# fwrnke/pseudo-3D-interpolation

Hardware: AMD Instinct MI355X
Metric: POCS iterations/s on the 1024x1024x512 cube (higher is better)
Workload: dtype complex64 (f32 arithmetic)

## Files before the change

### include/p3d.h

```cpp
#ifndef P3D_H
#define P3D_H

#include <stddef.h>
#include <stdint.h>

#ifdef __cplusplus
extern "C" {
#endif

#define P3D_ABI_VERSION 1

#define P3D_OK 0
#define P3D_ERR_INVALID (-1)
#define P3D_ERR_UNSUPPORTED (-2)
#define P3D_ERR_HIP (-3)

#define P3D_C64 0
#define P3D_F32 1
#define P3D_C128 2
#define P3D_F64 3

#define P3D_OP_HARD 0
#define P3D_OP_SOFT 1
#define P3D_OP_GARROTE 2
#define P3D_OP_PERCENTILE 16

#define P3D_VER_REGULAR 0
#define P3D_VER_FAST 1
#define P3D_VER_ADAPTIVE 2

#define P3D_FLAG_PROFILE 1
#define P3D_FLAG_PRIMED 2
#define P3D_FLAG_MASK_PER_SLICE 4

typedef struct p3d_plan p3d_plan;

typedef struct p3d_pocs_params {
    int32_t niter;
    int32_t thresh_op;
    int32_t version;
    int32_t flags;
    double eps;
    double alpha;
} p3d_pocs_params;

#define P3D_STATS_PER_SLICE 6

int p3d_abi_version(void);
const char* p3d_last_error(void);
int p3d_runtime_info(int* compiled_hip_version, int* runtime_hip_version);
int p3d_device_count(int* n);

int p3d_shape_supported(int nil, int nxl);

int p3d_plan_create(p3d_plan** out, int device, int nil, int nxl, int max_slices);
int p3d_plan_destroy(p3d_plan* plan);

int p3d_malloc(p3d_plan* plan, void** dptr, size_t bytes);
int p3d_free(p3d_plan* plan, void* dptr);
int p3d_memcpy_h2d(p3d_plan* plan, void* dst_dev, const void* src_host, size_t bytes);
int p3d_memcpy_d2h(p3d_plan* plan, void* dst_host, const void* src_dev, size_t bytes);
int p3d_dev_malloc(int device, void** dptr, size_t bytes);
int p3d_dev_free(void* dptr);
int p3d_dev_memcpy(int device, void* dst, const void* src, size_t bytes, int kind);
int p3d_dev_memset(int device, void* dptr, int value, size_t bytes);
int p3d_dev_synchronize(int device);
int p3d_dev_mem_info(int device, size_t* free_bytes, size_t* total_bytes);
int p3d_host_alloc(void** hptr, size_t bytes);
int p3d_host_free(void* hptr);
int p3d_host_register(void* hptr, size_t bytes);
int p3d_host_unregister(void* hptr);

int p3d_fft2_c64_dev(p3d_plan* plan, const void* in_dev, void* out_dev, int nslices, int inverse);
int p3d_fft2_c64(p3d_plan* plan, const void* in_host, void* out_host, int nslices, int inverse);

int p3d_fft2_shrink_c64(p3d_plan* plan, const void* in_host, const double* tau, int thresh_op, void* out_host,
                        int nslices);

int p3d_pocs_stats_dev(p3d_plan* plan, const void* x_dev, int dtype, int nslices, double* stats_host);
int p3d_pocs_prime_dev(p3d_plan* plan, const void* x_dev, int dtype, const float* mask_dev, int nslices, double* stats_host);
int p3d_pocs_stats(p3d_plan* plan, const void* x_host, int dtype, int nslices, double* stats_host);

int p3d_pocs_sorted_spectrum(p3d_plan* plan, const void* x, int nslices, float* peaks_host);
int p3d_pocs_data_driven_pick(p3d_plan* plan, int nslices, int niter, const float* bounds_host, float* tau_host, int64_t* count_host);

int p3d_pocs_run_dev(p3d_plan* plan, const void* x_dev, int dtype, const float* mask_dev, const double* tau,
                     const uint8_t* active, const p3d_pocs_params* params, void* out_dev, int nslices,
                     int32_t* niter_done, double* sums, double* elapsed_ms);
int p3d_pocs_run(p3d_plan* plan, const void* x_host, int dtype, const float* mask_host, const double* tau,
                 const uint8_t* active, const p3d_pocs_params* params, void* out_host, int nslices,
                 int32_t* niter_done, double* sums, double* elapsed_ms);

int p3d_multi_stats(int ndev, const int* devices, int nil, int nxl, const void* x_host, int dtype, int nslices, double* stats_host);
int p3d_multi_run(int ndev, const int* devices, int nil, int nxl, const void* x_host, int dtype, const float* mask_host,
                  const double* tau, const uint8_t* active, const p3d_pocs_params* params, void* out_host, int nslices,
                  int32_t* niter_done, double* sums);

#define P3D_DCT_BACKWARD 0
#define P3D_DCT_ORTHO 1
int p3d_dct2_c64_dev(p3d_plan* plan, const void* in_dev, void* out_dev, int nslices, int inverse, int norm);
int p3d_dct2_c64(p3d_plan* plan, const void* in_host, void* out_host, int nslices, int inverse, int norm);
int p3d_dct_shrink_c64(p3d_plan* plan, const void* in_host, const double* tau, int thresh_op, void* out_host, int nslices, int norm);
int p3d_pocs_dct_stats_dev(p3d_plan* plan, const void* x_dev, int dtype, int nslices, double* stats_host, int norm);
int p3d_pocs_dct_stats(p3d_plan* plan, const void* x_host, int dtype, int nslices, double* stats_host, int norm);
int p3d_pocs_dct_run_dev(p3d_plan* plan, const void* x_dev, int dtype, const float* mask_dev, const double* tau, const uint8_t* active,
                         const p3d_pocs_params* params, void* out_dev, int nslices, int32_t* niter_done, double* sums,
                         double* elapsed_ms, int norm);
int p3d_pocs_dct_run(p3d_plan* plan, const void* x_host, int dtype, const float* mask_host, const double* tau, const uint8_t* active,
                     const p3d_pocs_params* params, void* out_host, int nslices, int32_t* niter_done, double* sums,
                     double* elapsed_ms, int norm);

typedef struct p3d_patch_plan p3d_patch_plan;
int p3d_patch_plan_create(p3d_patch_plan** out, p3d_plan* plan, int nil, int nxl, const int32_t* starts_il, int n_il, const int32_t* starts_xl,
                          int n_xl, const float* taper_il, const float* taper_xl, int max_slices);
int p3d_patch_plan_destroy(p3d_patch_plan* pplan);
int p3d_patch_plan_info(p3d_patch_plan* pplan, int* npatch, int* max_jobs, int* resident_shape);
int p3d_patch_gather_dev(p3d_patch_plan* pplan, const void* cube_dev, int dtype, int nslices, void* patches_dev);
int p3d_patch_mask_dev(p3d_patch_plan* pplan, const float* mask_dev, int mask_slices, int nslices, float* windows_dev, int* nonbinary);
int p3d_patch_route(p3d_patch_plan* pplan, const p3d_pocs_params* params, int* single_kernel);
int p3d_patch_run_dev(p3d_patch_plan* pplan, const void* patches_dev, int dtype, const double* tau, const uint8_t* active,
                      const p3d_pocs_params* params, void* out_dev, int nslices, int32_t* niter_done, double* sums, double* elapsed_ms);
int p3d_patch_dct_route(p3d_patch_plan* pplan, const p3d_pocs_params* params, int norm, int* single_kernel);
int p3d_patch_dct_run_dev(p3d_patch_plan* pplan, const void* patches_dev, int dtype, const double* tau, const uint8_t* active,
                          const p3d_pocs_params* params, int norm, void* out_dev, int nslices, int32_t* niter_done, double* sums, double* elapsed_ms);
int p3d_patch_blend_dev(p3d_patch_plan* pplan, const void* patches_dev, int dtype, const uint8_t* active, void* out_dev, int nslices);

typedef struct p3d_plan64 p3d_plan64;
int p3d_plan64_create(p3d_plan64** out, int device, int nil, int nxl, int max_slices);
int p3d_plan64_destroy(p3d_plan64* plan);
int p3d_pocs64_stats(p3d_plan64* plan, const void* x, int dtype, int nslices, double* stats_host);
int p3d_fft2_c128(p3d_plan64* plan, const void* in_host, void* out_host, int nslices, int inverse);
int p3d_pocs64_run(p3d_plan64* plan, const void* x, int dtype, const double* mask, const double* tau, const uint8_t* active,
                   const p3d_pocs_params* params, void* out, int nslices, int32_t* niter_done, double* sums, double* elapsed_ms);
int p3d_pocs64_percentile(p3d_plan64* plan, const void* spectrum_host_c128, int nslices, const double* perc_host, double* thr_host);
// ... 194 lines not shown
```

### pseudo-3d-interpolation_amd/_ffi.py

```python
import ctypes as C
import importlib.util
import os
import sys

import numpy as np

_HERE = os.path.dirname(os.path.abspath(__file__))
LIB_PATH = os.environ.get("P3D_LIB_PATH") or os.path.join(_HERE, "libp3d_hip.so")

P3D_OK = 0
P3D_ERR_INVALID, P3D_ERR_UNSUPPORTED, P3D_ERR_HIP = -1, -2, -3
P3D_C64, P3D_F32 = 0, 1
P3D_C128, P3D_F64 = 2, 3
P3D_OP = {"hard": 0, "soft": 1, "garrote": 2, "garotte": 2}
P3D_OP_PERCENTILE = 16
P3D_OP.update({f"{k}-percentile": v | P3D_OP_PERCENTILE for k, v in list(P3D_OP.items())})
P3D_VER = {"regular": 0, "fast": 1, "adaptive": 2}
P3D_FLAG_PROFILE = 1
P3D_FLAG_PRIMED = 2
P3D_FLAG_MASK_PER_SLICE = 4
STATS_PER_SLICE = 6
P3D_DCT_NORM = {None: 0, "backward": 0, "ortho": 1}


class P3DError(RuntimeError):
    def __init__(self, code, msg):
        super().__init__(f"libp3d_hip error {code}: {msg}")
        self.code = code


class UnsupportedError(P3DError, NotImplementedError):
    pass


class PocsParams(C.Structure):
    _fields_ = [("niter", C.c_int32), ("thresh_op", C.c_int32), ("version", C.c_int32), ("flags", C.c_int32),
                ("eps", C.c_double), ("alpha", C.c_double)]


_lib = None

PROTOTYPES = {
    "p3d_abi_version": (C.c_int, []),
    "p3d_last_error": (C.c_char_p, []),
    "p3d_device_count": (C.c_int, [C.POINTER(C.c_int)]),
    "p3d_shape_supported": (C.c_int, [C.c_int, C.c_int]),
    "p3d_plan_create": (C.c_int, [C.POINTER(C.c_void_p), C.c_int, C.c_int, C.c_int, C.c_int]),
    "p3d_plan_destroy": (C.c_int, [C.c_void_p]),
    "p3d_malloc": (C.c_int, [C.c_void_p, C.POINTER(C.c_void_p), C.c_size_t]),
    "p3d_free": (C.c_int, [C.c_void_p, C.c_void_p]),
    "p3d_host_alloc": (C.c_int, [C.POINTER(C.c_void_p), C.c_size_t]),
    "p3d_host_free": (C.c_int, [C.c_void_p]),
    "p3d_memcpy_h2d": (C.c_int, [C.c_void_p, C.c_void_p, C.c_void_p, C.c_size_t]),
    "p3d_memcpy_d2h": (C.c_int, [C.c_void_p, C.c_void_p, C.c_void_p, C.c_size_t]),
    "p3d_fft2_c64_dev": (C.c_int, [C.c_void_p, C.c_void_p, C.c_void_p, C.c_int, C.c_int]),
    "p3d_fft2_c64": (C.c_int, [C.c_void_p, C.c_void_p, C.c_void_p, C.c_int, C.c_int]),
    "p3d_fft2_shrink_c64": (C.c_int, [C.c_void_p, C.c_void_p, C.c_void_p, C.c_int, C.c_void_p, C.c_int]),
    "p3d_pocs_stats_dev": (C.c_int, [C.c_void_p, C.c_void_p, C.c_int, C.c_int, C.c_void_p]),
    "p3d_runtime_info": (C.c_int, [C.POINTER(C.c_int), C.POINTER(C.c_int)]),
    "p3d_plan64_create": (C.c_int, [C.POINTER(C.c_void_p), C.c_int, C.c_int, C.c_int, C.c_int]),
    "p3d_plan64_destroy": (C.c_int, [C.c_void_p]),
    "p3d_pocs64_stats": (C.c_int, [C.c_void_p, C.c_void_p, C.c_int, C.c_int, C.c_void_p]),
    "p3d_fft2_c128": (C.c_int, [C.c_void_p, C.c_void_p, C.c_void_p, C.c_int, C.c_int]),
    "p3d_pocs64_run": (C.c_int, [C.c_void_p, C.c_void_p, C.c_int, C.c_void_p, C.c_void_p, C.c_void_p, C.POINTER(PocsParams), C.c_void_p, C.c_int,
                                 C.c_void_p, C.c_void_p, C.POINTER(C.c_double)]),
    "p3d_pocs64_percentile": (C.c_int, [C.c_void_p, C.c_void_p, C.c_int, C.c_void_p, C.c_void_p]),
    "p3d_pocs64_sorted_spectrum": (C.c_int, [C.c_void_p, C.c_void_p, C.c_int, C.c_int, C.c_void_p]),
    "p3d_pocs64_data_driven_pick": (C.c_int, [C.c_void_p, C.c_int, C.c_int, C.c_void_p, C.c_void_p, C.c_void_p]),
    "p3d_dct2_c128": (C.c_int, [C.c_void_p, C.c_void_p, C.c_void_p, C.c_int, C.c_int, C.c_int]),
    "p3d_pocs64_dct_stats": (C.c_int, [C.c_void_p, C.c_void_p, C.c_int, C.c_int, C.c_void_p, C.c_int]),
    "p3d_pocs64_dct_run": (C.c_int, [C.c_void_p, C.c_void_p, C.c_int, C.c_void_p, C.c_void_p, C.c_void_p, C.POINTER(PocsParams), C.c_void_p, C.c_int,
                                     C.c_void_p, C.c_void_p, C.POINTER(C.c_double), C.c_int]),
    "p3d_dev_malloc": (C.c_int, [C.c_int, C.POINTER(C.c_void_p), C.c_size_t]),
    "p3d_dev_free": (C.c_int, [C.c_void_p]),
    "p3d_dev_memcpy": (C.c_int, [C.c_int, C.c_void_p, C.c_void_p, C.c_size_t, C.c_int]),
    "p3d_dev_memset": (C.c_int, [C.c_int, C.c_void_p, C.c_int, C.c_size_t]),
    "p3d_dev_synchronize": (C.c_int, [C.c_int]),
    "p3d_dev_mem_info": (C.c_int, [C.c_int, C.POINTER(C.c_size_t), C.POINTER(C.c_size_t)]),
    "p3d_host_register": (C.c_int, [C.c_void_p, C.c_size_t]),
    "p3d_host_unregister": (C.c_int, [C.c_void_p]),
    "p3d_pocs_prime_dev": (C.c_int, [C.c_void_p, C.c_void_p, C.c_int, C.c_void_p, C.c_int, C.c_void_p]),
    "p3d_pocs_stats": (C.c_int, [C.c_void_p, C.c_void_p, C.c_int, C.c_int, C.c_void_p]),
    "p3d_pocs_sorted_spectrum": (C.c_int, [C.c_void_p, C.c_void_p, C.c_int, C.c_void_p]),
    "p3d_pocs_data_driven_pick": (C.c_int, [C.c_void_p, C.c_int, C.c_int, C.c_void_p, C.c_void_p, C.c_void_p]),
    "p3d_pocs_run_dev": (C.c_int, [C.c_void_p, C.c_void_p, C.c_int, C.c_void_p, C.c_void_p, C.c_void_p,
                                   C.POINTER(PocsParams), C.c_void_p, C.c_int, C.c_void_p, C.c_void_p,
                                   C.POINTER(C.c_double)]),
    "p3d_dct2_c64_dev": (C.c_int, [C.c_void_p, C.c_void_p, C.c_void_p, C.c_int, C.c_int, C.c_int]),
    "p3d_dct2_c64": (C.c_int, [C.c_void_p, C.c_void_p, C.c_void_p, C.c_int, C.c_int, C.c_int]),
    "p3d_dct_shrink_c64": (C.c_int, [C.c_void_p, C.c_void_p, C.c_void_p, C.c_int, C.c_void_p, C.c_int, C.c_int]),
    "p3d_pocs_dct_stats_dev": (C.c_int, [C.c_void_p, C.c_void_p, C.c_int, C.c_int, C.c_void_p, C.c_int]),
    "p3d_pocs_dct_stats": (C.c_int, [C.c_void_p, C.c_void_p, C.c_int, C.c_int, C.c_void_p, C.c_int]),
    "p3d_pocs_dct_run_dev": (C.c_int, [C.c_void_p, C.c_void_p, C.c_int, C.c_void_p, C.c_void_p, C.c_void_p,
                                   C.POINTER(PocsParams), C.c_void_p, C.c_int, C.c_void_p, C.c_void_p,
                                   C.POINTER(C.c_double), C.c_int]),
    "p3d_pocs_dct_run": (C.c_int, [C.c_void_p, C.c_void_p, C.c_int, C.c_void_p, C.c_void_p, C.c_void_p,
                                   C.POINTER(PocsParams), C.c_void_p, C.c_int, C.c_void_p, C.c_void_p,
                                   C.POINTER(C.c_double), C.c_int]),
    "p3d_pocs_run": (C.c_int, [C.c_void_p, C.c_void_p, C.c_int, C.c_void_p, C.c_void_p, C.c_void_p,
                               C.POINTER(PocsParams), C.c_void_p, C.c_int, C.c_void_p, C.c_void_p,
                               C.POINTER(C.c_double)]),
    "p3d_patch_plan_create": (C.c_int, [C.POINTER(C.c_void_p), C.c_void_p, C.c_int, C.c_int, C.c_void_p, C.c_int, C.c_void_p, C.c_int, C.c_void_p, C.c_void_p,
                                        C.c_int]),
    "p3d_patch_plan_destroy": (C.c_int, [C.c_void_p]),
    "p3d_patch_plan_info": (C.c_int, [C.c_void_p, C.POINTER(C.c_int), C.POINTER(C.c_int), C.POINTER(C.c_int)]),
    "p3d_patch_gather_dev": (C.c_int, [C.c_void_p, C.c_void_p, C.c_int, C.c_int, C.c_void_p]),
    "p3d_patch_mask_dev": (C.c_int, [C.c_void_p, C.c_void_p, C.c_int, C.c_int, C.c_void_p, C.POINTER(C.c_int)]),
    "p3d_patch_route": (C.c_int, [C.c_void_p, C.POINTER(PocsParams), C.POINTER(C.c_int)]),
    "p3d_patch_run_dev": (C.c_int, [C.c_void_p, C.c_void_p, C.c_int, C.c_void_p, C.c_void_p, C.POINTER(PocsParams), C.c_void_p, C.c_int, C.c_void_p,
                                    C.c_void_p, C.POINTER(C.c_double)]),
    "p3d_patch_dct_route": (C.c_int, [C.c_void_p, C.POINTER(PocsParams), C.c_int, C.POINTER(C.c_int)]),
    "p3d_patch_dct_run_dev": (C.c_int, [C.c_void_p, C.c_void_p, C.c_int, C.c_void_p, C.c_void_p, C.POINTER(PocsParams), C.c_int, C.c_void_p, C.c_int, C.c_void_p,
                                        C.c_void_p, C.POINTER(C.c_double)]),
    "p3d_patch_blend_dev": (C.c_int, [C.c_void_p, C.c_void_p, C.c_int, C.c_void_p, C.c_void_p, C.c_int]),
    "p3d_multi_stats": (C.c_int, [C.c_int, C.c_void_p, C.c_int, C.c_int, C.c_void_p, C.c_int, C.c_int, C.c_void_p]),
    "p3d_multi_run": (C.c_int, [C.c_int, C.c_void_p, C.c_int, C.c_int, C.c_void_p, C.c_int, C.c_void_p, C.c_void_p, C.c_void_p,
                                C.POINTER(PocsParams), C.c_void_p, C.c_int, C.c_void_p, C.c_void_p]),
    "p3d_time2freq": (C.c_int, [C.c_int, C.c_void_p, C.c_int, C.c_size_t, C.c_double, C.c_double, C.c_int, C.c_int, C.c_void_p,
                                C.c_void_p]),
    "p3d_freq2time": (C.c_int, [C.c_int, C.c_void_p, C.c_int, C.c_void_p, C.c_size_t, C.c_double, C.c_double, C.c_int, C.c_int,
                                C.c_void_p]),
    "p3d_time2freq_dev": (C.c_int, [C.c_int, C.c_void_p, C.c_int, C.c_size_t, C.c_double, C.c_double, C.c_int, C.c_int, C.c_void_p,
                                    C.c_void_p]),
    "p3d_freq2time_dev": (C.c_int, [C.c_int, C.c_void_p, C.c_int, C.c_void_p, C.c_size_t, C.c_double, C.c_double, C.c_int, C.c_int,
                                    C.c_void_p]),
    "p3d_last_sparsity": (C.c_int, [C.c_void_p, C.POINTER(C.c_double)]),
    "p3d_smooth_gaussian": (C.c_int, [C.c_int, C.c_void_p, C.c_size_t, C.c_int, C.c_int, C.c_double, C.c_double, C.c_void_p]),
    "p3d_smooth_median": (C.c_int, [C.c_int, C.c_void_p, C.c_size_t, C.c_int, C.c_int, C.c_int, C.c_void_p]),
# ... 89 lines not shown
    "p3d_shearlet_transform_c64": (C.c_int, [C.c_void_p, C.c_void_p, C.c_void_p, C.c_int]),
    "p3d_shearlet_inverse_c64": (C.c_int, [C.c_void_p, C.c_void_p, C.c_void_p, C.c_int]),
    "p3d_shearlet_stats": (C.c_int, [C.c_void_p, C.c_void_p, C.c_int, C.c_int, C.c_void_p]),
    "p3d_shearlet_run": (C.c_int, [C.c_void_p, C.c_void_p, C.c_int, C.c_void_p, C.c_void_p, C.c_void_p, C.POINTER(PocsParams),
                                   C.c_void_p, C.c_int, C.c_void_p, C.c_void_p, C.POINTER(C.c_double)]),
}


def _preload_torch_hip():
    if not os.environ.get("P3D_TORCH_HIP_PRELOAD") or "torch" in sys.modules:
        return
    try:
        spec = importlib.util.find_spec("torch")
        path = os.path.join(os.path.dirname(spec.origin), "lib", "libamdhip64.so") if spec and spec.origin else None
        if path and os.path.isfile(path):
            C.CDLL(path, mode=C.RTLD_GLOBAL)
    except (ImportError, OSError, ValueError):
        pass


def lib():
    global _lib
    if _lib is None:
        if not os.path.isfile(LIB_PATH):
            raise ImportError(
                f"{LIB_PATH} not found: build it with `make -C {os.path.join(_HERE, 'csrc')}` "
                "(or python -c 'import __graft_entry__ as g; g.build()'). There is no CPU fallback.")
        _preload_torch_hip()
        handle = C.CDLL(LIB_PATH)
        for name, (res, args) in PROTOTYPES.items():
            fn = getattr(handle, name)
            fn.restype = res
            fn.argtypes = args
        _lib = handle
        _check_runtime(handle)
    return _lib


_runtime = None


def _check_runtime(handle):
    global _runtime
    comp, run = C.c_int(0), C.c_int(0)
    path = None
    try:
        if handle.p3d_runtime_info(C.byref(comp), C.byref(run)) != P3D_OK:
            return
        with open("/proc/self/maps") as fh:
            for line in fh:
                if "libamdhip64" in line:
                    path = line.split()[-1]
                    break
    except OSError:
        pass

    def split(v):
        return v // 10000000, (v // 100000) % 100, v % 100000
    _runtime = {"compiled_hip_version": "%d.%d.%d" % split(comp.value), "runtime_hip_version": "%d.%d.%d" % split(run.value), "runtime_library": path}
    if split(comp.value)[:2] != split(run.value)[:2]:
        import warnings
        warnings.warn(f"libp3d_hip.so was compiled against HIP {_runtime['compiled_hip_version']} but the process runs HIP "
                      f"{_runtime['runtime_hip_version']} ({path}): another copy of the runtime was mapped first (PyTorch imported before this package, or "
                      f"P3D_TORCH_HIP_PRELOAD=1); processes that do not need torch.cuda should load this package first", RuntimeWarning, stacklevel=3)


def runtime_info():
    lib()
    return dict(_runtime or {})


def check(code):
    if code != P3D_OK:
        msg = lib().p3d_last_error().decode("utf-8", "replace")
        raise (UnsupportedError if code == P3D_ERR_UNSUPPORTED else P3DError)(code, msg)


def device_count():
    n = C.c_int(0)
    check(lib().p3d_device_count(C.byref(n)))
    return n.value


def shape_supported(nil, nxl):
    return bool(lib().p3d_shape_supported(int(nil), int(nxl)))


def _ptr(a):
    return a.ctypes.data_as(C.c_void_p)


class DeviceBuffer:

    def __init__(self, plan, nbytes):
        self.plan, self.nbytes = plan, int(nbytes)
        p = C.c_void_p()
        check(lib().p3d_malloc(plan.handle, C.byref(p), self.nbytes))
        self.ptr = p.value

    def upload(self, arr):
        arr = np.ascontiguousarray(arr)
        assert arr.nbytes <= self.nbytes
        check(lib().p3d_memcpy_h2d(self.plan.handle, self.ptr, _ptr(arr), arr.nbytes))
        return self

    def download(self, shape, dtype):
        out = np.empty(shape, dtype)
        assert out.nbytes <= self.nbytes
        check(lib().p3d_memcpy_d2h(self.plan.handle, _ptr(out), self.ptr, out.nbytes))
        return out

    def download_into(self, arr):
        if not arr.flags.c_contiguous or arr.nbytes > self.nbytes:
            raise ValueError("destination must be C-contiguous and no larger than the buffer")
        check(lib().p3d_memcpy_d2h(self.plan.handle, _ptr(arr), self.ptr, arr.nbytes))
        return arr

    def free(self):
        if self.ptr:
            check(lib().p3d_free(self.plan.handle, self.ptr))
            self.ptr = None


def _tau_table(tau, shape):
    tau = np.broadcast_to(np.asarray(tau), shape)
    t = np.empty(tau.shape + (2,), np.float64)
    t[..., 0] = tau.real
    t[..., 1] = tau.imag if np.iscomplexobj(tau) else 0.0
    return t


def _filter_bank(wavelet):
    bank = wavelet if isinstance(wavelet, (tuple, list)) else wavelet_filters(wavelet)
    bank = [np.ascontiguousarray(b, dtype=np.float64) for b in bank]
    if len(bank) != 4 or len({b.size for b in bank}) != 1:
        raise ValueError("a filter bank is (dec_lo, dec_hi, rec_lo, rec_hi) of equal length")
    return bank


def _real_psi(psi):
    psi = np.asarray(psi)
    if psi.ndim != 3:
        raise ValueError(f"Psi must be (nil, nxl, nshearlets), got shape {psi.shape}")
    if np.iscomplexobj(psi):
        raise NotImplementedError("complex shearlet spectra (realCoefficients=False) are not implemented")
    return psi


class _PlanBase:
    _DESTROY = _RUN = None
    _MASK_DT = np.float32

    def close(self):
        if getattr(self, "handle", None):
            getattr(lib(), self._DESTROY)(self.handle)
            self.handle = None

    def __del__(self):
        if lib is not None:
            self.close()

    def __enter__(self):
        return self

    def __exit__(self, *exc):
        self.close()
# ... 1410 lines not shown
```

### pseudo-3d-interpolation_amd/csrc/p3d_api.hip

```cpp
#include <hip/hip_runtime.h>

#include <climits>
#include <cmath>
#include <algorithm>
#include <cstdlib>
#include <cstring>
#include <string>
#include <thread>
#include <vector>

#include "p3d.h"
#include "p3d_dct.hpp"
#include "p3d_dct_tables.hpp"
#include "p3d_generic.hpp"
#include "p3d_host.hpp"
#include "p3d_internal.hpp"
#include "p3d_flex.hpp"
#include "p3d_mix_entry.hpp"
#include "p3d_resident.hpp"
#include "p3d_resident_dct.hpp"
#include "p3d_select.hpp"
#include "p3d_kernels.hpp"

namespace p3d {
// ... 280 lines not shown
    unsigned long long* nzl = nullptr;
    unsigned* cbase = nullptr;
    unsigned long long* mbits = nullptr;
    unsigned* mbase = nullptr;
    const p3d::mix::Entry* mix_row = nullptr;
    bool mix_binary = false;
    bool use32 = false;
    unsigned long long* bits32 = nullptr;
    c32* tw32 = nullptr;
    int* flag = nullptr;
    unsigned* rowbase = nullptr;
    char* xc = nullptr;
    size_t xc_cap = 0;
    double* sums = nullptr;
    size_t sums_cap = 0;
    double* rowsum = nullptr;
    c32* tau = nullptr;
    size_t tau_cap = 0;
    int* done = nullptr;
    float* partials = nullptr;
    int tiles = 0;
    int cus = 0;
    int pipe_wgs = 0;
    int host_sw = 0;
    int flex_over = 0;
    bool no_colpipe = false;
    void* st_x = nullptr;
    void* st_out = nullptr;
    float* st_mask = nullptr;
    size_t st_mask_cap = 0;
    size_t st_cap = 0;
    struct Primed { bool valid = false; const void* x = nullptr; const float* mask = nullptr; int dtype = 0, nslices = 0, nonbinary = 0, violation = 0; unsigned nobs = 0;
                    bool real = false;
    } primed;
    double* sum0 = nullptr;
    int sorted_slices = 0;
    c32* dct_w = nullptr;
    c32* dct_tab = nullptr;
    hipEvent_t ev0 = nullptr, ev1 = nullptr;
    std::vector<hipEvent_t> prof_events;
    double prof_col_ms = 0, prof_row_ms = 0;
    int prof_col_n = 0, prof_row_n = 0;

    size_t slice_elems() const { return (size_t)nil * nxl; }
};

static int upload_table(p3d_plan* p, const LineOps* ops, bool for_rows, int n, c32** dst)
{
    std::vector<c32> host;
    if (is_flex(ops)) {
        flex_build_table(n, host);
    } else {
        host.resize(for_rows ? (size_t)ops->row_tw_slots : (size_t)ops->col_tw_slots);
        if (for_rows) ops->build_row_tw(host.data());
        else ops->build_col_tw(host.data());
    }
    P3D_TRY(hipMalloc((void**)dst, sizeof(c32) * host.size()));
    P3D_TRY(hipMemcpy(*dst, host.data(), sizeof(c32) * host.size(), hipMemcpyHostToDevice));
    return P3D_OK;
}

extern "C" {

int p3d_abi_version(void) { return P3D_ABI_VERSION; }

const char* p3d_last_error(void) { return g_err.c_str(); }

int p3d_runtime_info(int* compiled_hip_version, int* runtime_hip_version)
{
    if (!compiled_hip_version || !runtime_hip_version) return fail(P3D_ERR_INVALID, "NULL argument");
    *compiled_hip_version = HIP_VERSION;
    P3D_TRY(hipRuntimeGetVersion(runtime_hip_version));
    return P3D_OK;
}

int p3d_device_count(int* n)
{
    if (!n) return fail(P3D_ERR_INVALID, "n is NULL");
    *n = 0;
    P3D_TRY(hipGetDeviceCount(n));
    return P3D_OK;
}

static bool generic_ok(int n) { return n >= 1 && n <= GEN_MAX_N && gen_make_plan(n).nf >= 0; }

int p3d_shape_supported(int nil, int nxl)
{
    if (find_ops(nil) != nullptr && find_ops(nxl) != nullptr) return 1;
    return (generic_ok(nil) && generic_ok(nxl)) ? 1 : 0;
}

int p3d_plan_destroy(p3d_plan* p)
{
    if (!p) return P3D_OK;
    if (p->pct_plan) p3d_plan_destroy(p->pct_plan);
    hipSetDevice(p->device);
    if (p->stream) hipStreamSynchronize(p->stream);
    void* bufs[] = {p->mbits, p->mbase, p->cbase, p->bits64, p->bits32, p->tw32, p->nzl, p->nzflag, p->nzm, p->nzcount, p->tw_col, p->tw_row, p->work, p->bits, p->flag, p->rowbase, p->xc, p->sums, p->rowsum, p->sum0, p->tau, p->pct_sel, p->pct_hist, p->pct_frac, p->dct_w, p->dct_tab,
                    p->done,   p->partials, p->st_x, p->st_out, p->st_mask};
    for (void* b : bufs)
        if (b) hipFree(b);
    for (hipEvent_t e : p->prof_events) hipEventDestroy(e);
    if (p->ev0) hipEventDestroy(p->ev0);
    if (p->ev1) hipEventDestroy(p->ev1);
    if (p->stream) hipStreamDestroy(p->stream);
    delete p;
    return P3D_OK;
}

static int create_plan(p3d_plan** out, int device, int nil, int nxl, int max_slices, bool force_generic)
{
    if (!out) return fail(P3D_ERR_INVALID, "out is NULL");
    *out = nullptr;
    if (nil < 1 || nxl < 1 || max_slices < 1) return fail(P3D_ERR_INVALID, "nil, nxl and max_slices must be positive");
    if (max_slices > 65535) return fail(P3D_ERR_INVALID, "max_slices > 65535: split the cube into batches");
    const LineOps* oc = find_ops(nil);
    const LineOps* orow = find_ops(nxl);
    const bool generic = !oc || !orow || force_generic;
    if (generic && !(generic_ok(nil) && generic_ok(nxl)))
        return fail(P3D_ERR_UNSUPPORTED, "slice shape %d x %d: extents up to %d are supported", nil, nxl, GEN_MAX_N);
    if (int rc = use_device(device)) return rc;

    p3d_plan* p = new p3d_plan;
    p->device = device;
    p->nil = nil;
    p->nxl = nxl;
    p->max_slices = max_slices;
    p->generic = generic;
    p->ops_col = generic ? nullptr : oc;
    p->ops_row = generic ? nullptr : orow;
    p->host_sw = (getenv("P3D_FLEX_COL_NO_PERSIST") ? P3D_SW_FLEX_NO_PERSIST : 0) | (getenv("P3D_FLEX_NO_INPLACE") ? P3D_SW_FLEX_NO_INPLACE : 0);
    p->flex_over = getenv("P3D_FLEX_COL_OVER") ? atoi(getenv("P3D_FLEX_COL_OVER")) : 0;
    p->no_colpipe = getenv("P3D_NO_COLPIPE") != nullptr;
    if (generic) {
        p->gcol = gen_make_plan(nil);
        p->grow = gen_make_plan(nxl);
        p->tiles = p3d_plan::GEN_STAT_BLOCKS;
    } else {
        const int ct = is_flex(oc) ? flex_col_tile(nil) : oc->col_tile;
        p->tiles = (nxl + ct - 1) / ct;
        hipDeviceProp_t prop;
        P3D_TRY(hipGetDeviceProperties(&prop, device));
        p->cus = prop.multiProcessorCount;
        p->pipe_wgs = (orow->tpl > 0 && orow->tpl <= 256 && !getenv("P3D_NO_PIPE")) ? p->cus : 0;
    }
    int rc = P3D_OK;
    auto bail = [&](int code) {
        std::string keep = g_err;
        p3d_plan_destroy(p);
        g_err = keep;
        return code;
    };
#define TRY_OR_BAIL(expr)                                                                             \
    do {                                                                                              \
        hipError_t e_ = (expr);                                                                       \
        if (e_ != hipSuccess) {                                                                       \
            fail(P3D_ERR_HIP, "%s failed: %s", #expr, hipGetErrorString(e_));                         \
            return bail(P3D_ERR_HIP);                                                                 \
        }                                                                                             \
    } while (0)
    TRY_OR_BAIL(hipStreamCreateWithFlags(&p->stream, hipStreamNonBlocking));
    TRY_OR_BAIL(hipEventCreate(&p->ev0));
    TRY_OR_BAIL(hipEventCreate(&p->ev1));
    if (generic) {
        for (int which = 0; which < 2; ++which) {
            const int n = which ? nxl : nil;
// ... 1677 lines not shown
```

### pseudo-3d-interpolation_amd/csrc/p3d_fft32.hpp

```cpp
#pragma once

#include "p3d_fft.hpp"

namespace p3d {

struct P32 {
    static constexpr int N = 1024, ROWS = 16, THREADS = 512, UPB = 8;
    static constexpr int LSTR = 1024 + 2 * 32;
    static constexpr int TW = 31 * 32;
    static constexpr size_t lds_bytes() { return sizeof(c32) * (TW + (size_t)ROWS * LSTR); }
    static void build_tw(c32* out)
    {
        for (int t = 1; t < 32; ++t)
            for (int j = 0; j < 32; ++j) {
                const double ang = -6.283185307179586476925286766559 * double(t) * double(j) / 1024.0;
                out[(t - 1) * 32 + j] = c32{float(__builtin_cos(ang)), float(__builtin_sin(ang))};
            }
    }
};

template <int DIR>
P3D_HD c32 mul_tw(c32 a, c32 w) { return DIR > 0 ? mul_conj(a, w) : a * w; }

template <int DIR>
P3D_HD void dft16s(c32* a)
{
    constexpr float H = 0.70710678118654752440f, C = 0.92387953251128675613f, S = 0.38268343236508977173f;
    dft4<DIR>(a[0], a[4], a[8], a[12]);
    dft4<DIR>(a[1], a[5], a[9], a[13]);
    dft4<DIR>(a[2], a[6], a[10], a[14]);
    dft4<DIR>(a[3], a[7], a[11], a[15]);
    a[5] = mul_tw<DIR>(a[5], c32{C, -S});
    a[9] = mul_tw<DIR>(a[9], c32{H, -H});
    a[13] = mul_tw<DIR>(a[13], c32{S, -C});
    a[6] = mul_tw<DIR>(a[6], c32{H, -H});
    a[10] = mul_i<DIR>(a[10]);
    a[14] = mul_tw<DIR>(a[14], c32{-H, -H});
    a[7] = mul_tw<DIR>(a[7], c32{S, -C});
    a[11] = mul_tw<DIR>(a[11], c32{-H, -H});
    a[15] = mul_tw<DIR>(a[15], c32{-C, S});
    dft4<DIR>(a[0], a[1], a[2], a[3]);
    dft4<DIR>(a[4], a[5], a[6], a[7]);
    dft4<DIR>(a[8], a[9], a[10], a[11]);
    dft4<DIR>(a[12], a[13], a[14], a[15]);
}

template <int DIR>
P3D_HD void dft32(c32 (&x)[32])
{
    constexpr float C[8] = {1.0f, 0.98078528040323044913f, 0.92387953251128675613f, 0.83146961230254523708f, 0.70710678118654752440f, 0.55557023301960222474f,
                            0.38268343236508977173f, 0.19509032201612826785f};
    constexpr float S[8] = {0.0f, 0.19509032201612826785f, 0.38268343236508977173f, 0.55557023301960222474f, 0.70710678118654752440f, 0.83146961230254523708f,
                            0.92387953251128675613f, 0.98078528040323044913f};
    c32 e[16], o[16];
#pragma unroll
    for (int m = 0; m < 16; ++m) { e[m] = x[2 * m]; o[m] = x[2 * m + 1]; }
    dft16s<DIR>(e);
    dft16s<DIR>(o);
#pragma unroll
    for (int k = 0; k < 8; ++k) {
        const c32 ea = e[digit_rev<16>(k)], eb = e[digit_rev<16>(k + 8)];
        c32 oa = o[digit_rev<16>(k)], ob = o[digit_rev<16>(k + 8)];
        if (k != 0) {
            const c32 w{C[k], -S[k]};
            oa = mul_tw<DIR>(oa, w);
            ob = mul_tw<DIR>(ob, w);
        }
        x[k] = ea + oa;
        x[k + 16] = ea - oa;
        x[k + 8] = DIR > 0 ? add_ib(eb, ob) : sub_ib(eb, ob);
        x[k + 24] = DIR > 0 ? sub_ib(eb, ob) : add_ib(eb, ob);
    }
}

template <int DIR>
P3D_HD void p32_half1(c32 (&v)[32], c32* row, int j)
{
    dft32<DIR>(v);
    c32* const p = row + 34 * j;
#pragma unroll
    for (int m = 0; m < 32; ++m) p[m] = v[m];
}
template <int DIR>
P3D_HD void p32_half2(c32 (&v)[32], const c32* row, const c32* tw, int j)
{
    const c32* const q = row + j;
    v[0] = q[0];
#pragma unroll
    for (int t = 1; t < 32; ++t) {
        const c32 w = tw[(t - 1) * 32 + j];
        v[t] = DIR > 0 ? mul_conj(q[34 * t], w) : q[34 * t] * w;
    }
    dft32<DIR>(v);
}

}
```

Measured before the change: 420.0.

## Pipeline LDS reads in radix-32 second pass with paired ds_read2_b64 and staged waits

Replaces the per-element LDS loads of data and twiddles in the second radix-32 FFT pass with inline-asm ds_read2_b64 pairs, issued in four groups of eight. Explicit s_waitcnt lgkmcnt barriers let twiddle multiplies on one group run while later groups are still in flight. The aim is to halve LDS instruction count and hide LDS latency, at the cost of more live registers and fragile hand-scheduled asm. It also adds a small API for querying the device's CU count.

```diff
diff --git a/include/p3d.h b/include/p3d.h
--- a/include/p3d.h
+++ b/include/p3d.h
@@ -50,6 +50,7 @@
 const char* p3d_last_error(void);
 int p3d_runtime_info(int* compiled_hip_version, int* runtime_hip_version);
 int p3d_device_count(int* n);
+int p3d_device_cus(int device, int* n);
 
 int p3d_shape_supported(int nil, int nxl);
 
diff --git a/pseudo-3d-interpolation_amd/_ffi.py b/pseudo-3d-interpolation_amd/_ffi.py
--- a/pseudo-3d-interpolation_amd/_ffi.py
+++ b/pseudo-3d-interpolation_amd/_ffi.py
@@ -44,6 +44,7 @@
     "p3d_abi_version": (C.c_int, []),
     "p3d_last_error": (C.c_char_p, []),
     "p3d_device_count": (C.c_int, [C.POINTER(C.c_int)]),
+    "p3d_device_cus": (C.c_int, [C.c_int, C.POINTER(C.c_int)]),
     "p3d_shape_supported": (C.c_int, [C.c_int, C.c_int]),
     "p3d_plan_create": (C.c_int, [C.POINTER(C.c_void_p), C.c_int, C.c_int, C.c_int, C.c_int]),
     "p3d_plan_destroy": (C.c_int, [C.c_void_p]),
@@ -299,6 +300,12 @@
     return n.value
 
 
+def device_cus(device=0):
+    n = C.c_int(0)
+    check(lib().p3d_device_cus(int(device), C.byref(n)))
+    return n.value
+
+
 def shape_supported(nil, nxl):
     return bool(lib().p3d_shape_supported(int(nil), int(nxl)))
 
diff --git a/pseudo-3d-interpolation_amd/csrc/p3d_api.hip b/pseudo-3d-interpolation_amd/csrc/p3d_api.hip
--- a/pseudo-3d-interpolation_amd/csrc/p3d_api.hip
+++ b/pseudo-3d-interpolation_amd/csrc/p3d_api.hip
@@ -386,6 +386,14 @@
     return P3D_OK;
 }
 
+int p3d_device_cus(int device, int* n)
+{
+    if (!n) return fail(P3D_ERR_INVALID, "n is NULL");
+    *n = 0;
+    P3D_TRY(hipDeviceGetAttribute(n, hipDeviceAttributeMultiprocessorCount, device));
+    return P3D_OK;
+}
+
 static bool generic_ok(int n) { return n >= 1 && n <= GEN_MAX_N && gen_make_plan(n).nf >= 0; }
 
 int p3d_shape_supported(int nil, int nxl)
diff --git a/pseudo-3d-interpolation_amd/csrc/p3d_fft32.hpp b/pseudo-3d-interpolation_amd/csrc/p3d_fft32.hpp
--- a/pseudo-3d-interpolation_amd/csrc/p3d_fft32.hpp
+++ b/pseudo-3d-interpolation_amd/csrc/p3d_fft32.hpp
@@ -81,16 +81,80 @@
 #pragma unroll
     for (int m = 0; m < 32; ++m) p[m] = v[m];
 }
+#if defined(__HIP_DEVICE_COMPILE__)
+typedef float p32_two __attribute__((ext_vector_type(4)));
+__device__ __forceinline__ c32 p32_lo(p32_two r) { return c32{r.x, r.y}; }
+__device__ __forceinline__ c32 p32_hi(p32_two r) { return c32{r.z, r.w}; }
+template <int A, int B>
+__device__ __forceinline__ p32_two p32_read2(const c32* base)
+{
+    static_assert(A >= 0 && A < 256 && B >= 0 && B < 256, "ds_read2_b64 offsets");
+    const unsigned addr = (unsigned)(size_t)(const __attribute__((address_space(3))) c32*)base;
+    p32_two r;
+    asm volatile("ds_read2_b64 %0, %1 offset0:%2 offset1:%3" : "=v"(r) : "v"(addr), "n"(A), "n"(B) : "memory");
+    return r;
+}
+template <int LEFT>
+__device__ __forceinline__ void p32_arrived(p32_two (&a)[4], p32_two (&w)[4])
+{
+    __builtin_amdgcn_sched_barrier(0);
+    asm volatile("s_waitcnt lgkmcnt(%[left])"
+                 : "+v"(a[0]), "+v"(a[1]), "+v"(a[2]), "+v"(a[3]), "+v"(w[0]), "+v"(w[1]), "+v"(w[2]), "+v"(w[3])
+                 : [left] "n"(LEFT));
+}
+#else
+struct p32_two { c32 lo, hi; };
+inline c32 p32_lo(p32_two r) { return r.lo; }
+inline c32 p32_hi(p32_two r) { return r.hi; }
+template <int A, int B>
+inline p32_two p32_read2(const c32* base) { return p32_two{base[A], base[B]}; }
+template <int LEFT>
+inline void p32_arrived(p32_two (&)[4], p32_two (&)[4]) {}
+#endif
+template <int G>
+P3D_HD void p32_request(p32_two (&a)[4], p32_two (&w)[4], const c32* q, const c32* twj)
+{
+    const c32* const qb = q + 34 * 8 * G;
+    const c32* const wb = twj + (G == 0 ? 0 : 32 * (8 * G - 1));
+    constexpr int D = G == 0 ? -32 : 0;
+    a[0] = p32_read2<0, 34>(qb);
+    a[1] = p32_read2<68, 102>(qb);
+    a[2] = p32_read2<136, 170>(qb);
+    a[3] = p32_read2<204, 238>(qb);
+    w[0] = p32_read2<(D < 0 ? 0 : D), 32 + D>(wb);
+    w[1] = p32_read2<64 + D, 96 + D>(wb);
+    w[2] = p32_read2<128 + D, 160 + D>(wb);
+    w[3] = p32_read2<192 + D, 224 + D>(wb);
+}
+template <int DIR, int G>
+P3D_HD void p32_twiddle(c32 (&v)[32], const p32_two (&a)[4], const p32_two (&w)[4])
+{
+#pragma unroll
+    for (int i = 0; i < 4; ++i) {
+        const int t = 8 * G + 2 * i;
+        if (t == 0) v[0] = p32_lo(a[0]);
+        else v[t] = DIR > 0 ? mul_conj(p32_lo(a[i]), p32_lo(w[i])) : p32_lo(a[i]) * p32_lo(w[i]);
+        v[t + 1] = DIR > 0 ? mul_conj(p32_hi(a[i]), p32_hi(w[i])) : p32_hi(a[i]) * p32_hi(w[i]);
+    }
+}
 template <int DIR>
 P3D_HD void p32_half2(c32 (&v)[32], const c32* row, const c32* tw, int j)
 {
     const c32* const q = row + j;
-    v[0] = q[0];
-#pragma unroll
-    for (int t = 1; t < 32; ++t) {
-        const c32 w = tw[(t - 1) * 32 + j];
-        v[t] = DIR > 0 ? mul_conj(q[34 * t], w) : q[34 * t] * w;
-    }
+    const c32* const twj = tw + j;
+    p32_two a0[4], w0[4], a1[4], w1[4], a2[4], w2[4], a3[4], w3[4];
+    p32_request<0>(a0, w0, q, twj);
+    p32_request<1>(a1, w1, q, twj);
+    p32_arrived<8>(a0, w0);
+    p32_twiddle<DIR, 0>(v, a0, w0);
+    p32_request<2>(a2, w2, q, twj);
+    p32_arrived<8>(a1, w1);
+    p32_twiddle<DIR, 1>(v, a1, w1);
+    p32_request<3>(a3, w3, q, twj);
+    p32_arrived<8>(a2, w2);
+    p32_twiddle<DIR, 2>(v, a2, w2);
+    p32_arrived<0>(a3, w3);
+    p32_twiddle<DIR, 3>(v, a3, w3);
     dft32<DIR>(v);
 }
 
```

Result: faster. 431.1 (median of 6 runs) (+2.6%).
